# phylo42/IPK

Measured on AMD Instinct MI355X. Metric: scored phylo-k-mers/sec, higher is better.
Workload: dtype f32

## Files before the change

ipk_amd/csrc/ipkgpu.hip:

```cpp
#include <cstring>
#include <hip/hip_runtime.h>
#include <rocprim/rocprim.hpp>

#include <algorithm>
#include <cmath>
#include <cstdarg>
#include <cstdio>
#include <cstring>
#include <new>
#include <string>
#include <type_traits>
#include <unordered_map>
#include <memory>
#include <vector>

#include "../../include/ipkgpu.h"
#include "dcla_device.hpp"
#include "kernels_score.hpp"
#include "kernels_quad.hpp"
#include "kernels_compact.hpp"
#include "kernels_keymajor.hpp"
#include "kernels_reduce_pipe.hpp"
#include "kernels_filter.hpp"
#include "kernels_dbfile.hpp"
// ... 65 lines not shown
    hipStream_t stream = nullptr;
    std::string err;
    int64_t workspace_bytes = 0;
    int64_t opt_variant = 0;
    int64_t opt_flags = 0;
    int64_t opt_kmc_pass = 0;
    int64_t opt_slice = 0;
    uint64_t sliced_windows = 0;
    int64_t opt_prefix_mats = 0;
    int64_t opt_wg_chunks2 = 0;
    int64_t opt_rounds = 0;
    int64_t opt_pool_limit = 0;
    int64_t opt_pool_chunks = 0;
    DevBuf table, best, ovfq, counts, offsets, goff, idx, branch, scan_sums, scan_boff, tmp_a, tmp_b, tmp_c;
    DevBuf pool, desc, gbcnt, gboff, gbcur, clist, gm, tile_next;
    DevBuf ptrs;
    DevBuf sp_bits, sp_pops, sp_rank, sp_c16;
    void* h_spill[2] = {nullptr, nullptr}; hipEvent_t ev_spill[2] = {nullptr, nullptr}; size_t h_spill_cap = 0;
    size_t held = 0, held_peak = 0;
    int64_t budget = 0;
    size_t refused_need = 0;
    DevBuf mask;
    bool mask_valid = false;
    uint64_t mask_words = 0;
    bool table_compressed = false;
    DevBuf rank, vaddr, ucnt, qpack, xstart, pcounts;
    DevBuf seq, pvals, pvaddr, mrank, cursnap;
    DevBuf cvals, coff, croom;
    bool comp_own_vals = false;
    std::vector<uint32_t> h_branch;
    uint32_t comp_nb = 0, comp_stride = 0, comp_tbl = 0;
    double pairs_per_window = 0;
    uint64_t count_pass_pairs = 0;
    uint64_t count_pass_queued = 0;
    double acc_main_ms = 0, acc_reduce_ms = 0;
    double acc_count_ms = 0, acc_write_ms = 0, acc_km_ms = 0;
    const char* main_kernel = "";
    std::vector<std::pair<void*, size_t>> free_blocks;
    std::unordered_map<void*, size_t> live_blocks;
    size_t cached_bytes = 0, cache_limit = 0;
    void* small = nullptr;
    void* h_up = nullptr; size_t h_up_cap = 0; hipEvent_t up_done = nullptr; bool up_pending = false;
    unsigned long long emitted_host = 0; bool emitted_fetched = false;
    uint32_t* h_rb = nullptr;
    EventPool events;
    bool spec_skip_wait = false;
    uint64_t pool_want_min = 0;
    struct Pending {
        bool active = false;
        std::unique_ptr<Stopwatch> sw; int ev_a = -1, ev_b = -1, ev_c = -1, ev_d = -1;
        uint64_t cap = 0, max_chunks = 0, windows = 0; uint32_t gb = 0; bool pool_ovf_ok = false, use_quad = false;
    } pend;
    uint64_t last_entries = 0; uint32_t last_gb = 0;
    double t_write_total = 0, t_write_device = 0, t_write_file = 0;
    int64_t opt_load_chunk = 0;
    int64_t opt_load_window = 0;
    double t_load[10] = {0, 0, 0, 0, 0, 0, 0, 0, 0, 0};
    double t_diff_ms = 0;
    std::vector<uint64_t> dfiles_ranges;
    double dfiles_stat[12] = {0, 0, 0, 0, 0, 0, 0, 0, 0, 0, 0, 0};
    double t_select_ms = 0;
    int64_t opt_union_copy = 0;
    double t_union[4] = {0, 0, 0, 0};
    DevBuf place_seq, place_off, place_out, place_tables, place_small, place_amb;
    int64_t opt_place_batch = 0;
    int64_t opt_place_lds = 0;
// ... 214 lines not shown
        ctx->live_blocks[*out] = *got;
        ctx->cached_bytes -= *got;
        ctx->free_blocks.erase(ctx->free_blocks.begin() + best);
        return hipSuccess;
    }
    const hipError_t e = ctx_alloc(ctx, out, want_bytes);
    if (e == hipSuccess) *got = ctx->live_blocks[*out];
    return e;
}

static std::vector<DevBuf*> all_workspaces(ipkgpu_ctx* ctx)
{
    return {&ctx->table, &ctx->best, &ctx->ovfq, &ctx->counts, &ctx->offsets, &ctx->goff, &ctx->idx,
            &ctx->branch, &ctx->scan_sums, &ctx->scan_boff, &ctx->tmp_a, &ctx->tmp_b, &ctx->tmp_c,
            &ctx->pool, &ctx->desc, &ctx->gbcnt, &ctx->gboff, &ctx->gbcur, &ctx->clist, &ctx->gm, &ctx->tile_next, &ctx->mask,
            &ctx->rank, &ctx->vaddr, &ctx->ucnt, &ctx->qpack, &ctx->xstart, &ctx->pcounts, &ctx->ptrs,
            &ctx->cvals, &ctx->coff, &ctx->croom, &ctx->seq, &ctx->pvals, &ctx->pvaddr, &ctx->mrank, &ctx->cursnap,
            &ctx->sp_bits, &ctx->sp_pops, &ctx->sp_rank, &ctx->sp_c16,
            &ctx->place_seq, &ctx->place_off, &ctx->place_out, &ctx->place_tables, &ctx->place_small, &ctx->place_amb};
}

extern "C" {

uint32_t ipkgpu_bits_per_symbol(uint32_t sigma) { return sigma == 4 ? 2u : sigma == 20 ? 5u : 0u; }
uint32_t ipkgpu_max_k(uint32_t sigma) { return sigma == 4 ? 14u : sigma == 20 ? 6u : 0u; }
uint32_t ipkgpu_max_k_keyrange(uint32_t sigma) { return sigma == 4 ? 16u : ipkgpu_max_k(sigma); }
size_t ipkgpu_kmer_batch(uint32_t key, size_t n_ranges) { return n_ranges ? key % n_ranges : 0; }

float ipkgpu_log_threshold(float omega, uint32_t sigma, uint32_t k)
{
    return log10f(powf(omega / (float)sigma, (float)k));
// ... 232 lines not shown
}

template <int SIGMA, int K, PairLayout LAYOUT = PairLayout::PAIR8>
int launch_stream_overflow(ipkgpu_ctx* ctx, const StreamParams& sp)
{
    constexpr uint32_t TBL = stream_tbl<SIGMA, K>();
    if constexpr (TBL == 0 || ipow(SIGMA, K - K / 2) <= (uint32_t)fast_cap<SIGMA, K>()) {
        (void)ctx; (void)sp;
        return IPKGPU_OK;
    } else if constexpr (LAYOUT != PairLayout::PAIR8 && (TBL & (TBL - 1)) != 0) {
        (void)sp;
        return fail(ctx, IPKGPU_ERR_INVALID, "no 6-byte pair layout for this sigma/k");
    } else {
        constexpr uint32_t NB = (uint32_t)((ipow(SIGMA, K) + TBL - 1) / TBL);
        constexpr size_t lds = TileGeo<SIGMA, K, 1>::HEAD_BYTES + (size_t)wave_scratch_entries<SIGMA, K, big_capf<SIGMA, K>()>() * 8 +
                               (size_t)OVF_NW * 2 * NB * SUB * 4;
        static_assert(lds + 64 <= 160 * 1024, "big-list (stream) LDS budget");
        auto kern = score_overflow_stream_kernel<SIGMA, K, TBL, LAYOUT>;
        if (lds > 64 * 1024)
            HIP_TRY(ctx, hipFuncSetAttribute(reinterpret_cast<const void*>(kern), hipFuncAttributeMaxDynamicSharedMemorySize, (int)lds));
        const uint32_t per_cu = (uint32_t)std::max<size_t>(1, std::min<size_t>(32 / OVF_NW, (160 * 1024) / (lds + 64)));
        hipLaunchKernelGGL(kern, dim3(ctx->num_cu * per_cu), dim3(OVF_NW * 64), lds, ctx->stream, sp);
        HIP_TRY(ctx, hipGetLastError());
        return IPKGPU_OK;
    }
}

#ifndef IPK_RPIPE_DEFAULT
#define IPK_RPIPE_DEFAULT 1
#endif
#ifndef IPK_RPIPE_D
// ... 552 lines not shown
    pd.active = false;
    std::unique_ptr<Stopwatch> sw(pd.sw.release());
    const uint32_t n_ovf = ctx->h_rb[SMALL_OVF_COUNT / 4], pool_exhausted = ctx->h_rb[SMALL_POOL_OVF / 4];
    if (pool_exhausted) {
        if (pd.cap >= pd.max_chunks) {
            ctx->pool_want_min = 0;
            if (pd.gb > 1) return IPKGPU_RETRY_SMALLER;
            return fail(ctx, IPKGPU_ERR_NOMEM, "the pair pool of ONE branch group is exhausted at the device-memory limit");
        }
        ctx->pool_want_min = pd.cap * 2;
        return IPKGPU_RETRY_AGAIN;
    }
    ctx->pool_want_min = 0;
    memcpy(&ctx->emitted_host, ctx->h_rb + SMALL_EMITTED / 4, 8);
    ctx->emitted_fetched = true;
    ctx->spec_skip_wait = !(n_ovf > 0 && (uint64_t)n_ovf * IPK_OVF_POOL_RATIO >= pd.windows && pd.pool_ovf_ok);
    if (sw) { ctx->acc_main_ms += sw->ms(pd.ev_a, pd.ev_b); ctx->acc_reduce_ms += sw->ms(pd.ev_c, pd.ev_d); }
    return IPKGPU_OK;
}

int arm_capped(ipkgpu_ctx* ctx, uint32_t sigma, uint32_t k, ScoreParams& p)
{
    static_assert(SMALL_SLICED + 4 == SMALL_BIG_OVF, "the count and the flag are cleared and read together");
    const bool capped_lists = sigma == 4 && k >= 13;
    p.big_ovf = capped_lists ? small_at(ctx, SMALL_BIG_OVF) : nullptr;
    p.slice_lists = capped_lists && ctx->opt_slice ? 1u : 0u;
    if (capped_lists) HIP_TRY(ctx, hipMemsetAsync(p.big_ovf - 1, 0, 8, ctx->stream));
    return IPKGPU_OK;
}

int check_capped(ipkgpu_ctx* ctx, uint32_t k, const ScoreParams& p)
// ... 143 lines not shown
        HIP_TRY(ctx, hipMemcpyAsync(&so, p.ovf_count, 4, hipMemcpyDeviceToHost, ctx->stream));
        HIP_TRY(ctx, hipStreamSynchronize(ctx->stream));
        ctx->count_pass_pairs = se; ctx->count_pass_queued = so;
        const uint64_t s_windows = (uint64_t)slist.size() * pl.nwin;
        const double cap_pairs = 0.25 * (double)pl.geo.fast_cap * (double)pl.geo.fast_cap;
        if (s_windows) ctx->pairs_per_window = std::max(1.0, ((double)se + (double)so * cap_pairs) / (double)s_windows * 1.15);
    }
    const double ppw_est = ctx->pairs_per_window > 0 ? ctx->pairs_per_window : 256.0;
    if (!s_compress && pool_ovf_ok && ctx->opt_variant == 0 && pl.table_size >= (1u << 16) &&
        (double)windows * ppw_est < 0.5 * (double)gb * (double)pl.table_size)
        s_compress = true;
    if (!s_compress) {
        RC_TRY(ensure(ctx, ctx->table, (size_t)gb * pl.table_size * 4));
        p.table = ctx->table.p;
    }
    const size_t lds_bytes = use_quad ? pl.geo.quad_lds : pl.geo.stream_lds;
    const uint64_t wg_per_cu = std::max<uint64_t>(1, std::min<uint64_t>(32 / SNW, (160 * 1024) / std::max<size_t>(lds_bytes, 1)));
    const uint64_t slots = (uint64_t)ctx->num_cu * wg_per_cu;
    const uint32_t CH = chunk_pairs_rt(TBL);
    const uint64_t CHB = chunk_bytes_rt(TBL, ps.layout);
    const uint64_t expected_chunks = (uint64_t)((double)windows * ppw_est / CH);
#ifndef IPK_WG_CHUNKS2
#define IPK_WG_CHUNKS2 2
#endif
    const uint64_t wg_chunks2 = ctx->opt_wg_chunks2 > 0 ? (uint64_t)ctx->opt_wg_chunks2 : (uint64_t)IPK_WG_CHUNKS2;
    const uint64_t max_wg = std::max<uint64_t>(slots, expected_chunks * 2 / wg_chunks2 / ((uint64_t)SNW * NBK * SUB));
#ifndef IPK_ROUNDS
#define IPK_ROUNDS 8
#endif
    const uint64_t rounds = std::max<uint64_t>(1, std::min<uint64_t>(ctx->opt_rounds > 0 ? (uint64_t)ctx->opt_rounds : (uint64_t)IPK_ROUNDS, max_wg / slots));
// ... 27 lines not shown
        RC_TRY(ensure(ctx, ctx->pool, (cap + 1) * CHB));
        RC_TRY(ensure(ctx, ctx->desc, cap * 8));
        if (!forced) cap = std::min<uint64_t>(ctx->pool.cap / CHB - 1, ctx->desc.cap / 8);
        RC_TRY(ensure(ctx, ctx->gbcnt, 2 * n_gb * 4));
        uint32_t* const d_gbcur = ctx->gbcnt.as<uint32_t>() + n_gb;
        RC_TRY(ensure(ctx, ctx->gboff, (n_gb + 1) * 8));
        uint32_t* d_pool_next = small_at(ctx, SMALL_POOL_NEXT);
        uint32_t* d_pool_ovf = small_at(ctx, SMALL_POOL_OVF);
        const bool pre_ok = use_quad && n_waves * NBK + 1024 <= cap && !(ctx->opt_flags & 32);
        const uint32_t pre_chunks = pre_ok ? (uint32_t)(n_waves * NBK) : 0u;
        uint32_t* d_tile_next = nullptr;
        if (use_quad && !(ctx->opt_flags & 128) && ((uint64_t)nb * s_tiles_per_mat >= 4ull * gb * S || (ctx->opt_flags & 256))) {
            RC_TRY(ensure(ctx, ctx->tile_next, (size_t)gb * 4));
            d_tile_next = ctx->tile_next.as<uint32_t>();
        }
        hipLaunchKernelGGL(small_reset_kernel, dim3((std::max<uint32_t>(gb, SMALL_XP_TOO_BIG / 4) + 255) / 256), dim3(256), 0, ctx->stream,
                           reinterpret_cast<uint32_t*>(ctx->small), pre_chunks, d_tile_next, gb, S);
        HIP_TRY(ctx, hipGetLastError());
        HIP_TRY(ctx, hipMemsetAsync(ctx->desc.p, 0, cap * 8, ctx->stream));

        StreamParams sp;
        sp.logp = logp_dev; sp.best = ctx->best.as<float>();
        sp.gm_off = ctx->gm.as<uint32_t>(); sp.gm_list = ctx->gm.as<uint32_t>() + gb + 1;
        sp.sites = pl.sites; sp.nwin = pl.nwin; sp.tiles_per_mat = s_tiles_per_mat; sp.S = S;
        sp.eps = pl.eps;
        sp.pool = ctx->pool.as<uint2>(); sp.pool_cap = (uint32_t)cap; sp.pool_next = d_pool_next;
        sp.desc = ctx->desc.as<unsigned long long>(); sp.pool_ovf = d_pool_ovf;
        sp.emitted = p.emitted; sp.ovf_queue = p.ovf_queue; sp.ovf_count = p.ovf_count; sp.mat_slot = p.mat_slot;
        sp.flags = (uint32_t)(ctx->opt_flags);
        sp.pre_chunks = pre_chunks;
        sp.tile_next = d_tile_next;
        std::unique_ptr<Stopwatch> sw_own(new Stopwatch(ctx->stream, &ctx->events));
        Stopwatch& sw = *sw_own;
        const int ev_a = sw.mark();
        RC_TRY(pass1(sp, n_wg, false));
        const int ev_b = sw.mark();
        const bool spec = ctx->spec_skip_wait && !s_compress && !(ctx->opt_flags & 64);
        uint32_t n_ovf = 0;
        uint32_t h[2] = {0, 0};
        if (!spec) {
            HIP_TRY(ctx, hipMemcpyAsync(ctx->h_rb, ctx->small, SMALL_BYTES, hipMemcpyDeviceToHost, ctx->stream));
            HIP_TRY(ctx, hipStreamSynchronize(ctx->stream));
            n_ovf = ctx->h_rb[SMALL_OVF_COUNT / 4]; h[0] = ctx->h_rb[SMALL_POOL_NEXT / 4]; h[1] = ctx->h_rb[SMALL_POOL_OVF / 4];
        }
        const bool ovf_in_pool = n_ovf > 0 && ((uint64_t)n_ovf * IPK_OVF_POOL_RATIO >= windows || s_compress) && pool_ovf_ok;
        if (ovf_in_pool) {
            RC_TRY(ensure(ctx, ctx->tmp_a, (size_t)n_ovf * 8));
            RC_TRY(ensure(ctx, ctx->tmp_b, (size_t)n_ovf * 8));
            hipLaunchKernelGGL(ovf_group_keys_kernel, dim3((n_ovf + 255) / 256), dim3(256), 0, ctx->stream,
                               p.ovf_queue, n_ovf, p.mat_slot, ctx->tmp_a.as<unsigned long long>());
            HIP_TRY(ctx, hipGetLastError());
            size_t tmp_bytes = 0;
            HIP_TRY(ctx, rocprim::radix_sort_keys(nullptr, tmp_bytes, ctx->tmp_a.as<unsigned long long>(), ctx->tmp_b.as<unsigned long long>(),
                                                  (size_t)n_ovf, 0, 64, ctx->stream));
            RC_TRY(ensure(ctx, ctx->tmp_c, tmp_bytes));
            HIP_TRY(ctx, rocprim::radix_sort_keys(ctx->tmp_c.p, tmp_bytes, ctx->tmp_a.as<unsigned long long>(), ctx->tmp_b.as<unsigned long long>(),
                                                  (size_t)n_ovf, 0, 64, ctx->stream));
            StreamParams so = sp;
            so.ovf_queue = ctx->tmp_b.as<unsigned long long>();
            if (use_quad) so.emitted = small_at<unsigned long long>(ctx, SMALL_OVF_EMITTED);
            RC_TRY(with_sigma_k(ctx, pl.sigma, pl.k, [&](auto S_, auto K_) {
                if constexpr (quad_layout<S_, K_>() == PairLayout::PAIR6) { if (ps.layout == PairLayout::PAIR6) return launch_stream_overflow<S_, K_, PairLayout::PAIR6>(ctx, so); }
                if (ps.layout != PairLayout::PAIR8) return fail(ctx, IPKGPU_ERR_INVALID, "no big-list kernel for the pass' pool layout");
                return launch_stream_overflow<S_, K_>(ctx, so);
            }));
        }
        if (ovf_in_pool) {
            HIP_TRY(ctx, hipMemcpyAsync(ctx->h_rb, ctx->small, SMALL_BYTES, hipMemcpyDeviceToHost, ctx->stream));
            HIP_TRY(ctx, hipStreamSynchronize(ctx->stream));
            h[0] = ctx->h_rb[SMALL_POOL_NEXT / 4]; h[1] = ctx->h_rb[SMALL_POOL_OVF / 4];
        }
        if (h[1] != 0) {
            if (cap >= max_chunks) {
                if (gb > 1) return IPKGPU_RETRY_SMALLER;
                return fail(ctx, IPKGPU_ERR_NOMEM, "the pair pool of ONE branch group is exhausted at the device-memory limit");
            }
            want = std::max<uint64_t>(cap * 2, want);
            continue;
        }
        const uint32_t n_used = spec ? (uint32_t)cap : (uint32_t)std::min<uint64_t>(h[0], cap);
        const uint32_t* n_used_dev = spec ? d_pool_next : nullptr;
        HIP_TRY(ctx, hipMemsetAsync(ctx->gbcnt.p, 0, 2 * n_gb * 4, ctx->stream));
// ... 22 lines not shown
            RC_TRY(ensure(ctx, ctx->vaddr, (size_t)gb * (ctx->mask_words / 2) * 8));
            RC_TRY(ensure(ctx, ctx->ucnt, n_gb * 4));
        }
        if (n_used) {
            const uint64_t n_grid = spec ? std::min<uint64_t>(n_used, expected_chunks * 2 + n_waves * NBK + 4096) : n_used;
            hipLaunchKernelGGL(chunk_scatter_kernel, dim3((uint32_t)std::min<uint64_t>((n_grid + 255) / 256, 1u << 16)), dim3(256), 0, ctx->stream,
                               ctx->desc.as<unsigned long long>(), n_used, ctx->gboff.as<uint64_t>(), d_gbcur,
                               ctx->clist.as<uint2>(), n_used_dev);
            HIP_TRY(ctx, hipGetLastError());
        }
        const int ev_c = sw.mark();
        RC_TRY(with_sigma_k(ctx, pl.sigma, pl.k, [&](auto S_, auto K_) {
            return launch_stream_pass2<S_, K_>(ctx, (uint32_t)n_gb, pl.table_size, ctx->table.as<uint32_t>(), s_compress, ps.layout);
        }));
        const int ev_d = sw.mark();
        if ((spec || n_ovf > 0) && !ovf_in_pool)
            RC_TRY(with_sigma_k(ctx, pl.sigma, pl.k, [&](auto S_, auto K_) { return launch_overflow<S_, K_, false>(ctx, p); }));
        if (s_compress) {
            ctx->table_compressed = true; ctx->comp_own_vals = true;
            ctx->comp_nb = NBK; ctx->comp_stride = 1; ctx->comp_tbl = TBL;
        }
        ctx->mask_valid = true;
        ctx->main_kernel = use_quad ? "score_quad_kernel" : "score_stream_kernel";
        HIP_TRY(ctx, hipMemcpyAsync(ctx->h_rb, ctx->small, SMALL_BYTES, hipMemcpyDeviceToHost, ctx->stream));
        ipkgpu_ctx::Pending& pd = ctx->pend;
        pd.sw.reset(sw_own.release());
        pd.ev_a = ev_a; pd.ev_b = ev_b; pd.ev_c = ev_c; pd.ev_d = ev_d;
        pd.cap = cap; pd.max_chunks = max_chunks; pd.windows = windows; pd.gb = gb; pd.pool_ovf_ok = pool_ovf_ok; pd.use_quad = use_quad;
        pd.active = true;
        if (defer) return IPKGPU_OK;
        HIP_TRY(ctx, hipStreamSynchronize(ctx->stream));
        const int rcf = stream_batch_check(ctx);
        if (rcf == IPKGPU_RETRY_AGAIN) { want = std::max<uint64_t>(want, ctx->pool_want_min); continue; }
        return rcf;
    }
    return fail(ctx, IPKGPU_ERR_NOMEM, "pair pool could not be sized");
}

int score_batch_finish(ipkgpu_ctx* ctx, const Plan& pl, uint32_t g0, uint32_t gb, uint64_t* emitted_acc)
{
    if (ctx->pend.active) RC_TRY(stream_batch_check(ctx));
    unsigned long long e = ctx->emitted_host;
    if (!ctx->emitted_fetched) {
// ... 96 lines not shown

    ipkgpu_result* res = new (std::nothrow) ipkgpu_result();
    if (!res) return fail(ctx, IPKGPU_ERR_NOMEM, "out of host memory");
    res->ctx = ctx;
    res->group_ids = pl.group_ids;
    res->offsets.assign((size_t)n_groups + 1, 0);
    struct Guard { ipkgpu_result* r; ~Guard() { if (r) ipkgpu_result_free(r); } } guard{res};
    void** const arrays[3] = {(void**)&res->d_keys, (void**)&res->d_scores, (void**)&res->d_positions};
    const int n_arrays = positions ? 3 : 2;

    RC_TRY(ensure(ctx, ctx->counts, (size_t)(pl.gpb * cpg) * 4));
    RC_TRY(ensure(ctx, ctx->offsets, (size_t)(pl.gpb * cpg + 1) * 8));
    RC_TRY(ensure(ctx, ctx->goff, (size_t)(pl.gpb + 1) * 8));

    ctx->acc_main_ms = ctx->acc_reduce_ms = ctx->acc_count_ms = ctx->acc_write_ms = ctx->acc_km_ms = 0;
    Stopwatch sw(ctx->stream, &ctx->events);
    const int t_begin = sw.mark();
    RC_TRY(run_prefix(ctx, pl, logp_dev));
    const int t_pre = sw.mark();
    std::vector<std::pair<int, int>> ev_score, ev_compact;
    uint64_t total_entries = 0;
    uint32_t gpb_now = (uint32_t)pl.gpb, gb = 0;
    for (uint32_t g0 = 0; g0 < n_groups; g0 += gb) {
        gb = std::min<uint32_t>(gpb_now, n_groups - g0);
        const int s0 = sw.mark();
        const int rcb = score_batch(ctx, pl, logp_dev, g0, gb, &res->emitted);
        if (rcb == IPKGPU_RETRY_SMALLER) { gpb_now = std::max<uint32_t>(1, gb / 2); gb = 0; continue; }
        if (rcb) return rcb;
        const int s1 = sw.mark();
        ev_score.push_back({s0, s1});
// ... 311 lines not shown
    const uint64_t slots = (T + P - 1) / P;
    const uint32_t n_groups = pl.n_groups;

    ipkgpu_parts* parts = new (std::nothrow) ipkgpu_parts();
    if (!parts) return fail(ctx, IPKGPU_ERR_NOMEM, "out of host memory");
    parts->ctx = ctx; parts->n_owners = P; parts->slots = slots;
    parts->lead = lead; parts->key_base = key_base; parts->sigma = sigma; parts->k = k;
    parts->owner_off.assign((size_t)P + 1, 0);
    struct Guard { ipkgpu_parts* r; ~Guard() { if (r) ipkgpu_parts_free(r); } } guard{parts};

    RC_TRY(ensure(ctx, ctx->branch, (size_t)n_groups * 4));
    ctx->h_branch = pl.group_ids;
    HIP_TRY(ctx, hipMemcpyAsync(ctx->branch.p, ctx->h_branch.data(), (size_t)n_groups * 4, hipMemcpyHostToDevice, ctx->stream));

    ctx->acc_main_ms = ctx->acc_reduce_ms = ctx->acc_count_ms = ctx->acc_write_ms = ctx->acc_km_ms = 0;
    Stopwatch sw(ctx->stream, &ctx->events);
    const int t_begin = sw.mark();
    RC_TRY(run_prefix(ctx, pl, logp_dev));
    const int t_pre = sw.mark();
    std::vector<std::pair<int, int>> ev_score, ev_compact, ev_km;
    std::pair<int, int> ev_keys{-1, -1};

    struct Batch { uint32_t* counts = nullptr; uint2* entries = nullptr; uint2* pentries = nullptr; std::vector<uint64_t> owner_off; };
    std::vector<Batch> batches;
    auto free_batches = [&]() { for (auto& b : batches) { ctx_release(ctx, b.counts); ctx_release(ctx, b.entries); ctx_release(ctx, b.pentries); } batches.clear(); };
    struct BGuard { decltype(free_batches)& f; ~BGuard() { f(); } } bguard{free_batches};

    const uint64_t n_slots_all = (uint64_t)P * slots;
    uint32_t gpb_now = (uint32_t)pl.gpb, gb = 0;
    for (uint32_t g0 = 0; g0 < n_groups; g0 += gb) {
// ... 902 lines not shown

int ipkgpu_get_option(const ipkgpu_ctx* ctx, const char* name, int64_t* value)
{
    if (!ctx || !name || !value) return IPKGPU_ERR_INVALID;
    if (!strcmp(name, "workspace_bytes")) { *value = ctx->workspace_bytes; return IPKGPU_OK; }
    if (!strcmp(name, "device_budget_bytes")) { *value = ctx->budget; return IPKGPU_OK; }
    if (!strcmp(name, "last_refused_bytes")) { *value = (int64_t)ctx->refused_need; return IPKGPU_OK; }
    if (!strcmp(name, "slice_long_lists")) { *value = ctx->opt_slice; return IPKGPU_OK; }
    if (!strcmp(name, "db_load_chunk_bytes")) { *value = ctx->opt_load_chunk; return IPKGPU_OK; }
    if (!strcmp(name, "db_load_window_bytes")) { *value = ctx->opt_load_window; return IPKGPU_OK; }
    if (!strcmp(name, "place_batch_queries")) { *value = ctx->opt_place_batch; return IPKGPU_OK; }
    if (!strcmp(name, "place_lds_branches")) { *value = ctx->opt_place_lds; return IPKGPU_OK; }
    if (!strcmp(name, "debug_sliced_windows")) { *value = (int64_t)ctx->sliced_windows; return IPKGPU_OK; }
    if (!strcmp(name, "debug_count_pass_pairs")) { *value = (int64_t)ctx->count_pass_pairs; return IPKGPU_OK; }
    if (!strcmp(name, "debug_count_pass_queued")) { *value = (int64_t)ctx->count_pass_queued; return IPKGPU_OK; }
    if (!strcmp(name, "debug_pool_bytes")) { *value = (int64_t)ctx->pool.cap; return IPKGPU_OK; }
    return IPKGPU_ERR_INVALID;
}

int ipkgpu_mem_stats(ipkgpu_ctx* ctx, uint64_t* held, uint64_t* held_peak, int reset_peak)
{
    if (!ctx) return IPKGPU_ERR_INVALID;
    if (held) *held = ctx->held;
    if (held_peak) *held_peak = ctx->held_peak;
    if (reset_peak) ctx->held_peak = ctx->held;
    return IPKGPU_OK;
}

int ipkgpu_parts_spill(ipkgpu_ctx* ctx, ipkgpu_parts* parts, const char* dir, uint32_t piece, uint64_t* bytes_written)
{
// ... 206 lines not shown
```

ipk_amd/csrc/kernels_score.hpp:

```cpp
#pragma once
#include <type_traits>
#include "dcla_device.hpp"

namespace ipkgpu {


template <int SIGMA, int M>
__global__ __launch_bounds__(256) void prefix_max_kernel(const float* __restrict__ logp, uint32_t n_mats, uint32_t sites,
                                                         float* __restrict__ best)
{
    constexpr int CH = 2048 / M;
    constexpr int ROW = CH + 4;
    static_assert(M == 1 || M == 2 || M == 4 || M == 8, "matrices per workgroup");
    __shared__ __align__(16) float cmbuf[2][M][ROW];
    const uint32_t mat0 = blockIdx.x * M;
    const uint32_t mv = min((uint32_t)M, n_mats - mat0);
    const bool chain = threadIdx.x < mv;
    const uint32_t my = mat0 + (chain ? threadIdx.x : 0u);
    float* b = best + (size_t)my * (sites + 1);
    if (chain) b[0] = 0.0f;
    float carry = 0.0f;
    auto maxima = [&](uint32_t c0, float (*cmw)[ROW], uint32_t t0, uint32_t nt) {
        const uint32_t n = min((uint32_t)CH, sites - c0);
        for (uint32_t mm = 0; mm < mv; ++mm) {
// ... 183 lines not shown
        }
        if (!ok) {
            if (lane_id() == 0) {
                const uint32_t q = atomicAdd(p.ovf_count, 1u);
                p.ovf_queue[q] = ((unsigned long long)mat << 32) | (unsigned long long)(t0 + w);
            }
        }
    }
    if (lane_id() == 0 && emitted) atomicAdd(p.emitted, emitted);
}

#ifndef IPK_OVF_NW
#define IPK_OVF_NW 8
#endif
constexpr int OVF_NW = IPK_OVF_NW;
#ifndef IPK_OVF_UNCOND_OR
#define IPK_OVF_UNCOND_OR 0
#endif
#ifndef IPK_OVF_PEEK
#define IPK_OVF_PEEK 0
#endif
#ifndef IPK_OVF_NOPUT
#define IPK_OVF_NOPUT 0
#endif
constexpr int BIG_CAP_ENTRIES = 6144;
template <int SIGMA, int K> constexpr int big_capf()
{
    return (size_t)wave_scratch_entries<SIGMA, K, 1 << 30>() * 8 <= (size_t)136 * 1024 ? (1 << 30) : BIG_CAP_ENTRIES;
}

// ... 492 lines not shown
        const uint32_t id = cbase[b];
        if (id != CHUNK_NONE) p.desc[id] = ((unsigned long long)(g * NB + b / SUB) << 32) | (unsigned long long)min(cfill[b], CH);
    }
    if (lane == 0 && emitted) atomicAdd(p.emitted, emitted);
}

template <int SIGMA, int K, uint32_t TBL, PairLayout LAYOUT = PairLayout::PAIR8>
__global__ __launch_bounds__(OVF_NW * 64) void score_overflow_stream_kernel(StreamParams p)
{
    extern __shared__ __align__(16) unsigned char smem[];
    constexpr uint32_t CH = chunk_pairs<TBL>();
    constexpr int CAPF = big_capf<SIGMA, K>();
    constexpr uint32_t T = ipow(SIGMA, K);
    constexpr uint32_t NB = (T + TBL - 1) / TBL;
    using TG = TileGeo<SIGMA, K, 1>;
    __shared__ uint32_t sh_n[2];
    float* cols = reinterpret_cast<float*>(smem);
    float* best = cols + TG::COLS_F;
    uint2* scratch = reinterpret_cast<uint2*>(smem + TG::HEAD_BYTES);
    uint32_t* state_all = reinterpret_cast<uint32_t*>(scratch + wave_scratch_entries<SIGMA, K, CAPF>());
    const uint32_t n = *p.ovf_count;
    const uint32_t lane = lane_id(), wave = threadIdx.x >> 6;
    uint32_t* cbase = state_all + (size_t)wave * 2 * NB * SUB;
    uint32_t* cfill = cbase + NB * SUB;
    for (uint32_t b = lane; b < NB * SUB; b += 64) { cbase[b] = CHUNK_NONE; cfill[b] = CH; }
    Appender<TBL, NB, LAYOUT> app{p, cbase, cfill, 0u};
    bool have_group = false;
    unsigned long long emitted = 0;
    constexpr uint32_t mulR = ipow(SIGMA, K - K / 2);
    auto close_chunks = [&]() {
        wave_lds_sync();
        for (uint32_t b = lane; b < NB * SUB; b += 64) {
            const uint32_t id = cbase[b];
            if (id != CHUNK_NONE) p.desc[id] = ((unsigned long long)(app.g * NB + b / SUB) << 32) | (unsigned long long)min(cfill[b], CH);
            cbase[b] = CHUNK_NONE; cfill[b] = CH;
        }
        wave_lds_sync();
    };
    const uint32_t per = (n + gridDim.x - 1) / gridDim.x;
    const uint32_t q_lo = min(n, blockIdx.x * per), q_hi = min(n, q_lo + per);
    for (uint32_t q = q_lo; q < q_hi; ++q) {
        const unsigned long long e = p.ovf_queue[q];
        const uint32_t g = (uint32_t)(e >> 42), mat = (uint32_t)(e >> 21) & 0x1FFFFFu, start = (uint32_t)e & 0x1FFFFFu;
        if (have_group && g != app.g) close_chunks();
        app.g = g; have_group = true;
        __syncthreads();
        const float* src = p.logp + ((size_t)mat * p.sites + start) * SIGMA;
        for (uint32_t i = threadIdx.x; i < K * SIGMA; i += OVF_NW * 64) cols[i] = src[i];
        const float* bsrc = p.best + (size_t)mat * (p.sites + 1) + start;
        for (uint32_t i = threadIdx.x; i <= K; i += OVF_NW * 64) best[i] = bsrc[i];
        __syncthreads();
        const uint2 *L = scratch, *R = scratch + Geo<SIGMA, K / 2, CAPF>::CAPH;
        if (wave == 0) {
            WinCtx c{cols, best, 0};
            uint32_t nL = 0, nR = 0;
            const bool fits = build_halves<SIGMA, K, CAPF>(c, p.eps, scratch, L, nL, R, nR);
            if (!fits) { nL = 0; nR = 0; if (lane == 0 && p.big_ovf) atomicOr(p.big_ovf, 1u); }
            if (lane == 0) { sh_n[0] = nL; sh_n[1] = nR; }
        }
        __syncthreads();
        const uint32_t nL = sh_n[0], nR = sh_n[1];
        if (nL == 0 || nR == 0) continue;
        uint32_t cnt = 0;
        for (uint32_t i = wave; i < nL; i += OVF_NW) {
            const uint2 a = L[i];
            for (uint32_t jb = 0; jb < nR; jb += 128) {
                const uint32_t ja = jb + lane, jc = jb + 64 + lane;
                const bool va = ja < nR, vb = jc < nR;
                uint2 b0 = make_uint2(0, 0), b1 = b0;
                if (va) b0 = R[ja];
                if (vb) b1 = R[jc];
                const float s0 = __uint_as_float(a.y) + __uint_as_float(b0.y);
                const float s1 = __uint_as_float(a.y) + __uint_as_float(b1.y);
                const bool p0 = va && (s0 > p.eps), p1 = vb && (s1 > p.eps);
                cnt += (uint32_t)__popcll(__ballot(p0)) + (uint32_t)__popcll(__ballot(p1));
                app.append2(p0, a.x * mulR + b0.x, __float_as_uint(s0), p1, a.x * mulR + b1.x, __float_as_uint(s1));
            }
        }
        emitted += cnt;
    }
    if (have_group) close_chunks();
    if (lane == 0 && emitted) atomicAdd(p.emitted, emitted);
}

__global__ __launch_bounds__(256) void ovf_group_keys_kernel(const unsigned long long* __restrict__ queue, uint32_t n,
                                                             const uint32_t* __restrict__ mat_slot,
                                                             unsigned long long* __restrict__ out)
{
    const uint32_t i = blockIdx.x * 256 + threadIdx.x;
    if (i >= n) return;
    const unsigned long long e = queue[i];
    const uint32_t mat = (uint32_t)(e >> 32), start = (uint32_t)e;
    out[i] = ((unsigned long long)mat_slot[mat] << 42) | ((unsigned long long)mat << 21) | (unsigned long long)start;
}

__global__ __launch_bounds__(256) void chunk_hist_kernel(const unsigned long long* __restrict__ desc, uint32_t n,
                                                         uint32_t* __restrict__ cnt, unsigned long long* __restrict__ pairs,
                                                         uint32_t* __restrict__ gb_pairs ,
                                                         const uint32_t* __restrict__ n_dev = nullptr)
{
    __shared__ unsigned long long wsum[4];
    unsigned long long c = 0;
    if (n_dev) n = min(n, *n_dev);
    for (uint32_t i = blockIdx.x * 256 + threadIdx.x; i < n; i += gridDim.x * 256) {
        const unsigned long long d = desc[i];
        if ((uint32_t)d != 0u) {
            atomicAdd(&cnt[(uint32_t)(d >> 32)], 1u);
            if (gb_pairs) atomicAdd(&gb_pairs[(uint32_t)(d >> 32)], (uint32_t)d);
// ... 13 lines not shown
__global__ __launch_bounds__(256) void chunk_scatter_kernel(const unsigned long long* __restrict__ desc, uint32_t n,
                                                            const uint64_t* __restrict__ off, uint32_t* __restrict__ cur,
                                                            uint2* __restrict__ list, const uint32_t* __restrict__ n_dev = nullptr)
{
    if (n_dev) n = min(n, *n_dev);
    for (uint32_t i = blockIdx.x * 256 + threadIdx.x; i < n; i += gridDim.x * 256) {
        const unsigned long long d = desc[i];
        if ((uint32_t)d == 0u) continue;
        const uint32_t gb = (uint32_t)(d >> 32);
        list[off[gb] + atomicAdd(&cur[gb], 1u)] = make_uint2(i, (uint32_t)d);
    }
}

constexpr uint32_t SMALL_EMITTED = 0;
constexpr uint32_t SMALL_OVF_COUNT = 16;
constexpr uint32_t SMALL_POOL_NEXT = 32;
constexpr uint32_t SMALL_POOL_OVF = 36;
constexpr uint32_t SMALL_SLICED = 40;
constexpr uint32_t SMALL_BIG_OVF = 44;
constexpr uint32_t SMALL_OVF_EMITTED = 48;
constexpr uint32_t SMALL_XP_TOO_BIG = 56;
constexpr uint32_t SMALL_REC_BIG = 60;
constexpr uint32_t SMALL_BYTES = 64;

__global__ void small_reset_kernel(uint32_t* __restrict__ small, uint32_t pre_chunks, uint32_t* __restrict__ tile_next, uint32_t n_groups,
                                   uint32_t first_tile)
{
    const uint32_t i = blockIdx.x * blockDim.x + threadIdx.x;
    if (i < SMALL_XP_TOO_BIG / 4) small[i] = i == SMALL_POOL_NEXT / 4 ? pre_chunks : 0u;
    if (tile_next && i < n_groups) tile_next[i] = first_tile;
}

__device__ __forceinline__ void store_slice_mask(const uint32_t* tab, uint32_t nslots, uint32_t* mask_words, uint32_t nthreads)
{
    const uint32_t lane = lane_id(), wave = threadIdx.x >> 6, nwv = nthreads >> 6;
    const uint32_t nblk = (nslots + 63) / 64;
    const uint32_t bpw = (nblk + nwv - 1) / nwv;
    const uint32_t b_lo = min(nblk, wave * bpw), b_hi = min(nblk, b_lo + bpw);
    for (uint32_t b0 = b_lo; b0 < b_hi; b0 += 64) {
        const uint32_t nb = min(64u, b_hi - b0);
        uint64_t mine = 0;
#pragma unroll 4
        for (uint32_t j = 0; j < nb; ++j) {
            const uint32_t c = (b0 + j) * 64;
            const uint32_t v = (c + lane < nslots) ? tab[c + lane] : 0u;
// ... 839 lines not shown
```

Baseline: 147.0 billion.

## Group big-list overflow queue on device and stage emits in LDS with dynamic draws

Adds a device-side count/scan/scatter path that groups overflow queue entries by group slot, replacing the host-synchronized radix sort and removing a host round-trip so the pass can stay speculative. The big-list stream kernel now takes queue entries through an atomic work counter instead of static ranges, iterates R-columns outer with several L-rows unrolled inner, and stages passing pairs in an LDS buffer before appending in batches. This is meant to cut host syncs, load imbalance and append overhead. It costs extra LDS per wave, two extra kernel launches plus a scan, and a larger tmp buffer sized to windows.

```diff
diff --git a/ipk_amd/csrc/ipkgpu.hip b/ipk_amd/csrc/ipkgpu.hip
--- a/ipk_amd/csrc/ipkgpu.hip
+++ b/ipk_amd/csrc/ipkgpu.hip
@@ -103,6 +103,7 @@
     int64_t opt_pool_chunks = 0;
     DevBuf table, best, ovfq, counts, offsets, goff, idx, branch, scan_sums, scan_boff, tmp_a, tmp_b, tmp_c;
     DevBuf pool, desc, gbcnt, gboff, gbcur, clist, gm, tile_next;
+    DevBuf ovfg, ovfoff;
     DevBuf ptrs;
     DevBuf sp_bits, sp_pops, sp_rank, sp_c16;
     void* h_spill[2] = {nullptr, nullptr}; hipEvent_t ev_spill[2] = {nullptr, nullptr}; size_t h_spill_cap = 0;
@@ -122,6 +123,7 @@
     double pairs_per_window = 0;
     uint64_t count_pass_pairs = 0;
     uint64_t count_pass_queued = 0;
+    uint64_t big_list_queued = 0; int big_list_route = 0;
     double acc_main_ms = 0, acc_reduce_ms = 0;
     double acc_count_ms = 0, acc_write_ms = 0, acc_km_ms = 0;
     const char* main_kernel = "";
@@ -139,6 +141,7 @@
         bool active = false;
         std::unique_ptr<Stopwatch> sw; int ev_a = -1, ev_b = -1, ev_c = -1, ev_d = -1;
         uint64_t cap = 0, max_chunks = 0, windows = 0; uint32_t gb = 0; bool pool_ovf_ok = false, use_quad = false;
+        bool ovf_dev_pool = false; int ovf_route = 0;
     } pend;
     uint64_t last_entries = 0; uint32_t last_gb = 0;
     double t_write_total = 0, t_write_device = 0, t_write_file = 0;
@@ -383,7 +386,7 @@
     return {&ctx->table, &ctx->best, &ctx->ovfq, &ctx->counts, &ctx->offsets, &ctx->goff, &ctx->idx,
             &ctx->branch, &ctx->scan_sums, &ctx->scan_boff, &ctx->tmp_a, &ctx->tmp_b, &ctx->tmp_c,
             &ctx->pool, &ctx->desc, &ctx->gbcnt, &ctx->gboff, &ctx->gbcur, &ctx->clist, &ctx->gm, &ctx->tile_next, &ctx->mask,
-            &ctx->rank, &ctx->vaddr, &ctx->ucnt, &ctx->qpack, &ctx->xstart, &ctx->pcounts, &ctx->ptrs,
+            &ctx->ovfg, &ctx->ovfoff, &ctx->rank, &ctx->vaddr, &ctx->ucnt, &ctx->qpack, &ctx->xstart, &ctx->pcounts, &ctx->ptrs,
             &ctx->cvals, &ctx->coff, &ctx->croom, &ctx->seq, &ctx->pvals, &ctx->pvaddr, &ctx->mrank, &ctx->cursnap,
             &ctx->sp_bits, &ctx->sp_pops, &ctx->sp_rank, &ctx->sp_c16,
             &ctx->place_seq, &ctx->place_off, &ctx->place_out, &ctx->place_tables, &ctx->place_small, &ctx->place_amb};
@@ -646,7 +649,7 @@
     } else {
         constexpr uint32_t NB = (uint32_t)((ipow(SIGMA, K) + TBL - 1) / TBL);
         constexpr size_t lds = TileGeo<SIGMA, K, 1>::HEAD_BYTES + (size_t)wave_scratch_entries<SIGMA, K, big_capf<SIGMA, K>()>() * 8 +
-                               (size_t)OVF_NW * 2 * NB * SUB * 4;
+                               (size_t)OVF_NW * 2 * NB * SUB * 4 + (size_t)OVF_NW * OVF_STAGE * 8;
         static_assert(lds + 64 <= 160 * 1024, "big-list (stream) LDS budget");
         auto kern = score_overflow_stream_kernel<SIGMA, K, TBL, LAYOUT>;
         if (lds > 64 * 1024)
@@ -1229,7 +1232,9 @@
     ctx->pool_want_min = 0;
     memcpy(&ctx->emitted_host, ctx->h_rb + SMALL_EMITTED / 4, 8);
     ctx->emitted_fetched = true;
-    ctx->spec_skip_wait = !(n_ovf > 0 && (uint64_t)n_ovf * IPK_OVF_POOL_RATIO >= pd.windows && pd.pool_ovf_ok);
+    ctx->spec_skip_wait = pd.ovf_dev_pool || !(n_ovf > 0 && (uint64_t)n_ovf * IPK_OVF_POOL_RATIO >= pd.windows && pd.pool_ovf_ok);
+    ctx->big_list_queued += n_ovf;
+    if (n_ovf > 0) ctx->big_list_route = pd.ovf_route;
     if (sw) { ctx->acc_main_ms += sw->ms(pd.ev_a, pd.ev_b); ctx->acc_reduce_ms += sw->ms(pd.ev_c, pd.ev_d); }
     return IPKGPU_OK;
 }
@@ -1403,6 +1408,8 @@
         RC_TRY(ensure(ctx, ctx->table, (size_t)gb * pl.table_size * 4));
         p.table = ctx->table.p;
     }
+    const bool ovf_dev_pool = !s_compress && pool_ovf_ok && !ps.positions && windows < (1ull << 32) && ctx->opt_variant != 99 &&
+                              !(ctx->opt_flags & 65536);
     const size_t lds_bytes = use_quad ? pl.geo.quad_lds : pl.geo.stream_lds;
     const uint64_t wg_per_cu = std::max<uint64_t>(1, std::min<uint64_t>(32 / SNW, (160 * 1024) / std::max<size_t>(lds_bytes, 1)));
     const uint64_t slots = (uint64_t)ctx->num_cu * wg_per_cu;
@@ -1460,8 +1467,15 @@
             RC_TRY(ensure(ctx, ctx->tile_next, (size_t)gb * 4));
             d_tile_next = ctx->tile_next.as<uint32_t>();
         }
+        uint32_t* d_ovf_groups = nullptr;
+        if (ovf_dev_pool) {
+            RC_TRY(ensure(ctx, ctx->ovfg, (size_t)gb * 2 * 4));
+            RC_TRY(ensure(ctx, ctx->ovfoff, ((size_t)gb + 1) * 8));
+            RC_TRY(ensure(ctx, ctx->tmp_b, (size_t)std::max<uint64_t>(windows, 1) * 8));
+            d_ovf_groups = ctx->ovfg.as<uint32_t>();
+        }
         hipLaunchKernelGGL(small_reset_kernel, dim3((std::max<uint32_t>(gb, SMALL_XP_TOO_BIG / 4) + 255) / 256), dim3(256), 0, ctx->stream,
-                           reinterpret_cast<uint32_t*>(ctx->small), pre_chunks, d_tile_next, gb, S);
+                           reinterpret_cast<uint32_t*>(ctx->small), pre_chunks, d_tile_next, gb, S, d_ovf_groups);
         HIP_TRY(ctx, hipGetLastError());
         HIP_TRY(ctx, hipMemsetAsync(ctx->desc.p, 0, cap * 8, ctx->stream));
 
@@ -1489,8 +1503,34 @@
             HIP_TRY(ctx, hipStreamSynchronize(ctx->stream));
             n_ovf = ctx->h_rb[SMALL_OVF_COUNT / 4]; h[0] = ctx->h_rb[SMALL_POOL_NEXT / 4]; h[1] = ctx->h_rb[SMALL_POOL_OVF / 4];
         }
-        const bool ovf_in_pool = n_ovf > 0 && ((uint64_t)n_ovf * IPK_OVF_POOL_RATIO >= windows || s_compress) && pool_ovf_ok;
-        if (ovf_in_pool) {
+        auto pool_kernel = [&](const unsigned long long* grouped) {
+            StreamParams so = sp;
+            so.ovf_queue = const_cast<unsigned long long*>(grouped);
+            if (use_quad) so.emitted = small_at<unsigned long long>(ctx, SMALL_OVF_EMITTED);
+            return with_sigma_k(ctx, pl.sigma, pl.k, [&](auto S_, auto K_) {
+                if constexpr (quad_layout<S_, K_>() == PairLayout::PAIR6) { if (ps.layout == PairLayout::PAIR6) return launch_stream_overflow<S_, K_, PairLayout::PAIR6>(ctx, so); }
+                if (ps.layout != PairLayout::PAIR8) return fail(ctx, IPKGPU_ERR_INVALID, "no big-list kernel for the pass' pool layout");
+                return launch_stream_overflow<S_, K_>(ctx, so);
+            });
+        };
+        const bool ovf_grouped = ovf_dev_pool && (spec || n_ovf > 0) && h[1] == 0;
+        if (ovf_grouped) {
+            const uint32_t q_cap = (uint32_t)windows;
+            const uint32_t q_grid = (uint32_t)std::min<uint64_t>(((uint64_t)q_cap + 255) / 256, (uint64_t)ctx->num_cu * 4);
+            uint32_t* const gcnt = ctx->ovfg.as<uint32_t>();
+            hipLaunchKernelGGL(ovf_group_count_kernel, dim3(q_grid), dim3(256), 0, ctx->stream,
+                               p.ovf_queue, p.ovf_count, q_cap, p.mat_slot, gcnt);
+            HIP_TRY(ctx, hipGetLastError());
+            RC_TRY(scan_u32(ctx, gcnt, gb, ctx->ovfoff.as<uint64_t>()));
+            hipLaunchKernelGGL(ovf_group_scatter_kernel, dim3(q_grid), dim3(256), 0, ctx->stream,
+                               p.ovf_queue, p.ovf_count, q_cap, p.mat_slot, ctx->ovfoff.as<uint64_t>(), gcnt + gb,
+                               ctx->tmp_b.as<unsigned long long>());
+            HIP_TRY(ctx, hipGetLastError());
+            RC_TRY(pool_kernel(ctx->tmp_b.as<unsigned long long>()));
+        }
+        const bool ovf_sorted = !ovf_dev_pool && n_ovf > 0 && pool_ovf_ok &&
+                                (s_compress || ((uint64_t)n_ovf * IPK_OVF_POOL_RATIO >= windows && !(ctx->opt_flags & 65536)));
+        if (ovf_sorted) {
             RC_TRY(ensure(ctx, ctx->tmp_a, (size_t)n_ovf * 8));
             RC_TRY(ensure(ctx, ctx->tmp_b, (size_t)n_ovf * 8));
             hipLaunchKernelGGL(ovf_group_keys_kernel, dim3((n_ovf + 255) / 256), dim3(256), 0, ctx->stream,
@@ -1502,16 +1542,10 @@
             RC_TRY(ensure(ctx, ctx->tmp_c, tmp_bytes));
             HIP_TRY(ctx, rocprim::radix_sort_keys(ctx->tmp_c.p, tmp_bytes, ctx->tmp_a.as<unsigned long long>(), ctx->tmp_b.as<unsigned long long>(),
                                                   (size_t)n_ovf, 0, 64, ctx->stream));
-            StreamParams so = sp;
-            so.ovf_queue = ctx->tmp_b.as<unsigned long long>();
-            if (use_quad) so.emitted = small_at<unsigned long long>(ctx, SMALL_OVF_EMITTED);
-            RC_TRY(with_sigma_k(ctx, pl.sigma, pl.k, [&](auto S_, auto K_) {
-                if constexpr (quad_layout<S_, K_>() == PairLayout::PAIR6) { if (ps.layout == PairLayout::PAIR6) return launch_stream_overflow<S_, K_, PairLayout::PAIR6>(ctx, so); }
-                if (ps.layout != PairLayout::PAIR8) return fail(ctx, IPKGPU_ERR_INVALID, "no big-list kernel for the pass' pool layout");
-                return launch_stream_overflow<S_, K_>(ctx, so);
-            }));
-        }
-        if (ovf_in_pool) {
+            RC_TRY(pool_kernel(ctx->tmp_b.as<unsigned long long>()));
+        }
+        const bool ovf_in_pool = ovf_grouped || ovf_sorted;
+        if (ovf_in_pool && !spec) {
             HIP_TRY(ctx, hipMemcpyAsync(ctx->h_rb, ctx->small, SMALL_BYTES, hipMemcpyDeviceToHost, ctx->stream));
             HIP_TRY(ctx, hipStreamSynchronize(ctx->stream));
             h[0] = ctx->h_rb[SMALL_POOL_NEXT / 4]; h[1] = ctx->h_rb[SMALL_POOL_OVF / 4];
@@ -1564,7 +1598,8 @@
             return launch_stream_pass2<S_, K_>(ctx, (uint32_t)n_gb, pl.table_size, ctx->table.as<uint32_t>(), s_compress, ps.layout);
         }));
         const int ev_d = sw.mark();
-        if ((spec || n_ovf > 0) && !ovf_in_pool)
+        const bool ovf_atomic = (spec || n_ovf > 0) && !ovf_in_pool;
+        if (ovf_atomic)
             RC_TRY(with_sigma_k(ctx, pl.sigma, pl.k, [&](auto S_, auto K_) { return launch_overflow<S_, K_, false>(ctx, p); }));
         if (s_compress) {
             ctx->table_compressed = true; ctx->comp_own_vals = true;
@@ -1577,6 +1612,7 @@
         pd.sw.reset(sw_own.release());
         pd.ev_a = ev_a; pd.ev_b = ev_b; pd.ev_c = ev_c; pd.ev_d = ev_d;
         pd.cap = cap; pd.max_chunks = max_chunks; pd.windows = windows; pd.gb = gb; pd.pool_ovf_ok = pool_ovf_ok; pd.use_quad = use_quad;
+        pd.ovf_dev_pool = ovf_dev_pool; pd.ovf_route = ovf_in_pool ? 2 : ovf_atomic ? 1 : 0;
         pd.active = true;
         if (defer) return IPKGPU_OK;
         HIP_TRY(ctx, hipStreamSynchronize(ctx->stream));
@@ -1703,6 +1739,7 @@
     RC_TRY(ensure(ctx, ctx->goff, (size_t)(pl.gpb + 1) * 8));
 
     ctx->acc_main_ms = ctx->acc_reduce_ms = ctx->acc_count_ms = ctx->acc_write_ms = ctx->acc_km_ms = 0;
+    ctx->big_list_queued = 0; ctx->big_list_route = 0;
     Stopwatch sw(ctx->stream, &ctx->events);
     const int t_begin = sw.mark();
     RC_TRY(run_prefix(ctx, pl, logp_dev));
@@ -2044,6 +2081,7 @@
     HIP_TRY(ctx, hipMemcpyAsync(ctx->branch.p, ctx->h_branch.data(), (size_t)n_groups * 4, hipMemcpyHostToDevice, ctx->stream));
 
     ctx->acc_main_ms = ctx->acc_reduce_ms = ctx->acc_count_ms = ctx->acc_write_ms = ctx->acc_km_ms = 0;
+    ctx->big_list_queued = 0; ctx->big_list_route = 0;
     Stopwatch sw(ctx->stream, &ctx->events);
     const int t_begin = sw.mark();
     RC_TRY(run_prefix(ctx, pl, logp_dev));
@@ -2976,6 +3014,8 @@
     if (!strcmp(name, "debug_sliced_windows")) { *value = (int64_t)ctx->sliced_windows; return IPKGPU_OK; }
     if (!strcmp(name, "debug_count_pass_pairs")) { *value = (int64_t)ctx->count_pass_pairs; return IPKGPU_OK; }
     if (!strcmp(name, "debug_count_pass_queued")) { *value = (int64_t)ctx->count_pass_queued; return IPKGPU_OK; }
+    if (!strcmp(name, "debug_big_list_route")) { *value = (int64_t)ctx->big_list_route; return IPKGPU_OK; }
+    if (!strcmp(name, "debug_big_list_queued")) { *value = (int64_t)ctx->big_list_queued; return IPKGPU_OK; }
     if (!strcmp(name, "debug_pool_bytes")) { *value = (int64_t)ctx->pool.cap; return IPKGPU_OK; }
     return IPKGPU_ERR_INVALID;
 }
diff --git a/ipk_amd/csrc/kernels_score.hpp b/ipk_amd/csrc/kernels_score.hpp
--- a/ipk_amd/csrc/kernels_score.hpp
+++ b/ipk_amd/csrc/kernels_score.hpp
@@ -221,6 +221,14 @@
 #define IPK_OVF_NW 8
 #endif
 constexpr int OVF_NW = IPK_OVF_NW;
+#ifndef IPK_OVF_DRAW_MIN
+#define IPK_OVF_DRAW_MIN 4
+#endif
+#ifndef IPK_OVF_DRAW_MAX
+#define IPK_OVF_DRAW_MAX 8
+#endif
+constexpr uint32_t OVF_DRAW_MIN = IPK_OVF_DRAW_MIN, OVF_DRAW_MAX = IPK_OVF_DRAW_MAX;
+constexpr uint32_t OVF_STAGE = 128;
 #ifndef IPK_OVF_UNCOND_OR
 #define IPK_OVF_UNCOND_OR 0
 #endif
@@ -743,12 +751,13 @@
     constexpr uint32_t T = ipow(SIGMA, K);
     constexpr uint32_t NB = (T + TBL - 1) / TBL;
     using TG = TileGeo<SIGMA, K, 1>;
-    __shared__ uint32_t sh_n[2];
+    __shared__ uint32_t sh_n[3];
     float* cols = reinterpret_cast<float*>(smem);
     float* best = cols + TG::COLS_F;
     uint2* scratch = reinterpret_cast<uint2*>(smem + TG::HEAD_BYTES);
     uint32_t* state_all = reinterpret_cast<uint32_t*>(scratch + wave_scratch_entries<SIGMA, K, CAPF>());
     const uint32_t n = *p.ovf_count;
+    if (n == 0) return;
     const uint32_t lane = lane_id(), wave = threadIdx.x >> 6;
     uint32_t* cbase = state_all + (size_t)wave * 2 * NB * SUB;
     uint32_t* cfill = cbase + NB * SUB;
@@ -757,7 +766,21 @@
     bool have_group = false;
     unsigned long long emitted = 0;
     constexpr uint32_t mulR = ipow(SIGMA, K - K / 2);
+    uint2* stage = reinterpret_cast<uint2*>(state_all + (size_t)OVF_NW * 2 * NB * SUB) + (size_t)wave * OVF_STAGE;
+    uint32_t staged = 0;
+    auto flush = [&]() {
+        if (staged == 0) return;
+        wave_lds_sync();
+        const bool p0 = lane < staged, p1 = lane + 64 < staged;
+        uint2 e0 = make_uint2(0, 0), e1 = e0;
+        if (p0) e0 = stage[lane];
+        if (p1) e1 = stage[lane + 64];
+        app.append2(p0, e0.x, e0.y, p1, e1.x, e1.y);
+        staged = 0;
+        wave_lds_sync();
+    };
     auto close_chunks = [&]() {
+        flush();
         wave_lds_sync();
         for (uint32_t b = lane; b < NB * SUB; b += 64) {
             const uint32_t id = cbase[b];
@@ -766,8 +789,14 @@
         }
         wave_lds_sync();
     };
-    const uint32_t per = (n + gridDim.x - 1) / gridDim.x;
-    const uint32_t q_lo = min(n, blockIdx.x * per), q_hi = min(n, q_lo + per);
+    uint32_t* const q_next = p.ovf_count + 1;
+    const bool spread = n <= gridDim.x;
+    const uint32_t run = spread ? 1u : min(OVF_DRAW_MAX, max(OVF_DRAW_MIN, (n + gridDim.x - 1) / gridDim.x));
+    for (;;) {
+    if (threadIdx.x == 0) sh_n[2] = atomicAdd(q_next, run);
+    __syncthreads();
+    const uint32_t q_lo = sh_n[2], q_hi = min(n, q_lo + run);
+    if (q_lo >= n) break;
     for (uint32_t q = q_lo; q < q_hi; ++q) {
         const unsigned long long e = p.ovf_queue[q];
         const uint32_t g = (uint32_t)(e >> 42), mat = (uint32_t)(e >> 21) & 0x1FFFFFu, start = (uint32_t)e & 0x1FFFFFu;
@@ -788,25 +817,40 @@
             if (lane == 0) { sh_n[0] = nL; sh_n[1] = nR; }
         }
         __syncthreads();
-        const uint32_t nL = sh_n[0], nR = sh_n[1];
+        const uint32_t nL = (uint32_t)__builtin_amdgcn_readfirstlane((int)sh_n[0]), nR = (uint32_t)__builtin_amdgcn_readfirstlane((int)sh_n[1]);
         if (nL == 0 || nR == 0) continue;
         uint32_t cnt = 0;
-        for (uint32_t i = wave; i < nL; i += OVF_NW) {
-            const uint2 a = L[i];
-            for (uint32_t jb = 0; jb < nR; jb += 128) {
-                const uint32_t ja = jb + lane, jc = jb + 64 + lane;
-                const bool va = ja < nR, vb = jc < nR;
-                uint2 b0 = make_uint2(0, 0), b1 = b0;
-                if (va) b0 = R[ja];
-                if (vb) b1 = R[jc];
-                const float s0 = __uint_as_float(a.y) + __uint_as_float(b0.y);
-                const float s1 = __uint_as_float(a.y) + __uint_as_float(b1.y);
-                const bool p0 = va && (s0 > p.eps), p1 = vb && (s1 > p.eps);
-                cnt += (uint32_t)__popcll(__ballot(p0)) + (uint32_t)__popcll(__ballot(p1));
-                app.append2(p0, a.x * mulR + b0.x, __float_as_uint(s0), p1, a.x * mulR + b1.x, __float_as_uint(s1));
+        constexpr uint32_t OVF_ROWS = 4;
+        const uint32_t r_step = spread ? (uint32_t)OVF_NW : 1u;
+        const uint32_t r_lo = (uint32_t)__builtin_amdgcn_readfirstlane((int)(spread ? wave : (nL * wave) / OVF_NW));
+        const uint32_t r_cnt = (uint32_t)__builtin_amdgcn_readfirstlane((int)(spread ? (nL + OVF_NW - 1 - wave) / OVF_NW
+                                                                                     : (nL * (wave + 1)) / OVF_NW - (nL * wave) / OVF_NW));
+        for (uint32_t jb = 0; jb < nR; jb += 64) {
+            const uint32_t j = jb + lane;
+            const bool valid = j < nR;
+            uint2 b = make_uint2(0, 0);
+            if (valid) b = R[j];
+            const float by = __uint_as_float(b.y);
+            for (uint32_t t0 = 0; t0 < r_cnt; t0 += OVF_ROWS) {
+                uint2 a[OVF_ROWS];
+#pragma unroll
+                for (uint32_t u = 0; u < OVF_ROWS; ++u) a[u] = L[r_lo + min(t0 + u, r_cnt - 1) * r_step];
+#pragma unroll
+                for (uint32_t u = 0; u < OVF_ROWS; ++u) {
+                    const float s = __uint_as_float(a[u].y) + by;
+                    const bool pass = valid && (t0 + u < r_cnt) && (s > p.eps);
+                    const uint64_t m = __ballot(pass);
+                    if (m != 0) {
+                        const uint32_t np = (uint32_t)__popcll(m);
+                        if (staged + np > OVF_STAGE) flush();
+                        if (pass) stage[staged + mbcnt(m)] = make_uint2(a[u].x * mulR + b.x, __float_as_uint(s));
+                        staged += np; cnt += np;
+                    }
+                }
             }
         }
         emitted += cnt;
+    }
     }
     if (have_group) close_chunks();
     if (lane == 0 && emitted) atomicAdd(p.emitted, emitted);
@@ -821,6 +865,27 @@
     const unsigned long long e = queue[i];
     const uint32_t mat = (uint32_t)(e >> 32), start = (uint32_t)e;
     out[i] = ((unsigned long long)mat_slot[mat] << 42) | ((unsigned long long)mat << 21) | (unsigned long long)start;
+}
+
+__global__ __launch_bounds__(256) void ovf_group_count_kernel(const unsigned long long* __restrict__ queue, const uint32_t* __restrict__ n_dev,
+                                                              uint32_t cap, const uint32_t* __restrict__ mat_slot, uint32_t* __restrict__ gcnt)
+{
+    const uint32_t n = min(*n_dev, cap);
+    for (uint32_t i = blockIdx.x * 256 + threadIdx.x; i < n; i += gridDim.x * 256)
+        atomicAdd(&gcnt[mat_slot[(uint32_t)(queue[i] >> 32)]], 1u);
+}
+__global__ __launch_bounds__(256) void ovf_group_scatter_kernel(const unsigned long long* __restrict__ queue, const uint32_t* __restrict__ n_dev,
+                                                                uint32_t cap, const uint32_t* __restrict__ mat_slot,
+                                                                const uint64_t* __restrict__ goff, uint32_t* __restrict__ gcur,
+                                                                unsigned long long* __restrict__ out)
+{
+    const uint32_t n = min(*n_dev, cap);
+    for (uint32_t i = blockIdx.x * 256 + threadIdx.x; i < n; i += gridDim.x * 256) {
+        const unsigned long long e = queue[i];
+        const uint32_t mat = (uint32_t)(e >> 32), start = (uint32_t)e, g = mat_slot[mat];
+        const uint64_t at = goff[g] + atomicAdd(&gcur[g], 1u);
+        if (at < cap) out[at] = ((unsigned long long)g << 42) | ((unsigned long long)mat << 21) | (unsigned long long)start;
+    }
 }
 
 __global__ __launch_bounds__(256) void chunk_hist_kernel(const unsigned long long* __restrict__ desc, uint32_t n,
@@ -864,6 +929,8 @@
 
 constexpr uint32_t SMALL_EMITTED = 0;
 constexpr uint32_t SMALL_OVF_COUNT = 16;
+constexpr uint32_t SMALL_OVF_NEXT = 20;
+static_assert(SMALL_OVF_COUNT + 4 == SMALL_OVF_NEXT, "score_overflow_stream_kernel finds the counter behind the length");
 constexpr uint32_t SMALL_POOL_NEXT = 32;
 constexpr uint32_t SMALL_POOL_OVF = 36;
 constexpr uint32_t SMALL_SLICED = 40;
@@ -874,11 +941,12 @@
 constexpr uint32_t SMALL_BYTES = 64;
 
 __global__ void small_reset_kernel(uint32_t* __restrict__ small, uint32_t pre_chunks, uint32_t* __restrict__ tile_next, uint32_t n_groups,
-                                   uint32_t first_tile)
+                                   uint32_t first_tile, uint32_t* __restrict__ ovf_groups = nullptr)
 {
     const uint32_t i = blockIdx.x * blockDim.x + threadIdx.x;
     if (i < SMALL_XP_TOO_BIG / 4) small[i] = i == SMALL_POOL_NEXT / 4 ? pre_chunks : 0u;
     if (tile_next && i < n_groups) tile_next[i] = first_tile;
+    if (ovf_groups && i < n_groups) { ovf_groups[i] = 0u; ovf_groups[n_groups + i] = 0u; }
 }
 
 __device__ __forceinline__ void store_slice_mask(const uint32_t* tab, uint32_t nslots, uint32_t* mask_words, uint32_t nthreads)
```

New measurement: 147.7 billion, median of 6. No clear change (+0.5%).
